# brayano/MultivarTV

Hardware: AMD Instinct MI355X
Metric: ADMM iters/sec on 512^3 fp64 mesh; achieved HBM GB/s vs peak at 1/2/4/8 GPUs (higher is better)
Workload: dtype f64; 1 GPU; 3D 512^3 fp64 mesh-TV ADMM, variant B (rcpp admm_update), lambda=1.0, fixed-iteration mode; theta_solver=spectral, nodes=134217728, edges=936381439, parallelism=single GPU

## Files before the change

### multivartv_amd/csrc/mvtv_admm3d.hip

```cpp
#include <algorithm>
#include <cstdlib>
#include <type_traits>

#include "mvtv_device.h"

namespace mvtv {

namespace e3d {
constexpr int TX = 64;
}

struct Edge3dArgs {
    Geom g;
    const double* theta;
    double* edges;
    const double* theta_old;
    double* g_alpha;
    double* g_u;
    const double* g_uprev;
    double* partials;
    double t_old, c_old, t_new;
    double t, c_prev;
    const AdmmCtl* ctl;
    int tiles_x, tiles_y, zchunk, nblocks;
// ... 316 lines not shown
    return pick(std::integral_constant<int, 256>{});
}

struct Fused3dArgs {
    Geom g;
    const double* theta;
    const double* z_old;
    double* z_new;
    const double* theta_old;
    double* g_alpha;
    double* g_u;
    const double* g_uprev;
    double* partials;
    double t_old, c_old, t_new, c_prev;
    const AdmmCtl* ctl;
    int tiles_x, tiles_y, zchunk, nblocks, zlo, zhi;
    int tpz;
    int xcd;
    int fold;
};

namespace f3a {
constexpr int IW = 65, IH = 15, TY = IH - 1, NT = 1024;
}

template <int NB, int ORD>
__host__ __device__ constexpr int f3a_nimg() {
    int n = 0;
    for (int k = 0; k < NB; ++k)
        if ((sprime_mask(block_code(k, 3, ORD), 3) & 3) != 0) ++n;
    return n;
}
template <int NB, int ORD>
__host__ __device__ constexpr int f3a_slot(int k) {
    int n = 0;
    for (int j = 0; j < k; ++j)
        if ((sprime_mask(block_code(j, 3, ORD), 3) & 3) != 0) ++n;
    return (sprime_mask(block_code(k, 3, ORD), 3) & 3) != 0 ? n : -1;
}

template <int ORD, int UM, bool DTH, int NB, bool TW>
__device__ __forceinline__ void admm3a_tile(const Fused3dArgs& a, double* __restrict__ szr, double (&red)[7], int X0,
                                            int Yh, int z0, int z1, double t_old, double c_old, double t_new,
                                            double c_prev, double rho_f) {
    constexpr int P = 3, NC = 8, IW = f3a::IW, IH = f3a::IH, NI = f3a_nimg<NB, ORD>();
    static_assert(!TW || twin_block(NB, P, ORD) >= 0, "twin blocks");
    const Geom& g = a.g;
    const int wv = int(threadIdx.x) >> 6, ln = int(threadIdx.x) & 63;
    const bool hcol = wv == IH;
    const int row = hcol ? ln : wv;
    const int col = hcol ? 0 : ln + 1;
    const int x = hcol ? X0 - 1 : X0 + ln, y = Yh + row;
    const int m0 = int(g.m[0]), m1 = int(g.m[1]), m2 = int(g.m[2]);
    const bool active = row < IH;
    const bool cell = active && x >= 0 && y >= 0 && x < m0 && y < m1;
    const bool inner = cell && !hcol && row > 0;
    const uint32_t pl = uint32_t(m0) * uint32_t(m1);
    const int xc = min(max(x, 0), m0 - 1), yc = min(max(y, 0), m1 - 1);
    const uint32_t xo[2] = {uint32_t(xc), uint32_t(min(xc + 1, m0 - 1))};
    const uint32_t yo[2] = {uint32_t(yc) * uint32_t(m0), uint32_t(min(yc + 1, m1 - 1)) * uint32_t(m0)};
    const uint32_t ixy = yo[0] + xo[0];
    const bool okx = x > 0, oky = y > 0;
    const bool hrow = row == 0;
    auto sidx = [&](int buf, int slot, int r, int c) { return ((buf * NI + slot) * IH + r) * IW + c; };

    auto load_theta = [&](double (&th)[4], int e) {
        const uint32_t zo = uint32_t(e) * pl;
#pragma unroll
        for (int q = 0; q < 4; ++q) th[q] = cell ? a.theta[zo + yo[q >> 1] + xo[q & 1]] : 0.0;
    };
    auto load_z = [&](double (&zo)[NB], int e) {
        const uint32_t i = uint32_t(e) * pl + ixy;
        static_for<0, NB>([&](auto kc) {
            constexpr int k = decltype(kc)::value;
            constexpr int S = sprime_mask(block_code(k, P, ORD), P);
            const bool need = cell && (!hrow || (S & 2)) && (!hcol || (S & 1));
            if constexpr (TW && twin_of(k, P, ORD) != k) zo[k] = 0.0;
            else zo[k] = need ? a.z_old[eix(g, k, i)] : 0.0;
        });
    };
    auto edge_cell = [&](int e, const double (&th0)[4], const double (&th1)[4], const double (&zo)[NB],
                         double (&zn)[NB], bool own) {
        const uint32_t i = uint32_t(e) * pl + ixy;
        double v[NC];
#pragma unroll
        for (int q = 0; q < 4; ++q) {
            v[q] = th0[q];
            v[q | 4] = th1[q];
        }
        if constexpr (DTH)
            if (own) red[3] = fmax(red[3], fabs(v[0] - a.theta_old[i]));
#pragma unroll
// ... 37 lines not shown
        constexpr int SI = S & 3;
        constexpr int sl = f3a_slot<NB, ORD>(k);
        qa = 0.0;
        qu = 0.0;
#pragma unroll
        for (int q = 0; q < 4; ++q) {
            if ((q & ~SI) != 0) continue;
            double v;
            if (q == 0) {
                v = own_z;
            } else {
                const bool ok = (!(q & 1) || okx) && (!(q & 2) || oky);
                if constexpr (sl >= 0) v = ok ? szr[sidx(buf, sl, row - ((q >> 1) & 1), col - (q & 1))] : 0.0;
                else v = 0.0;
            }
            const bool neg = __builtin_popcount(q) & 1;
            const double cl = clampd(v, t_new);
            const double al = v - cl;
            qa = neg ? qa - al : qa + al;
            qu = neg ? qu + cl : qu - cl;
        }
    };
    double qa_prev = 0.0, qu_prev = 0.0;
    double th0[4], th1[4], zo[NB], zn[NB];
    if (z0 > 0) {
        load_theta(th0, z0 - 1);
        load_theta(th1, z0);
        load_z(zo, z0 - 1);
        edge_cell(z0 - 1, th0, th1, zo, zn, false);
        to_image(1, zn);
        lds_barrier();
        if (inner) {
            static_for<0, NB>([&](auto kc) {
                constexpr int k = decltype(kc)::value;
                constexpr int S = sprime_mask(block_code(k, P, ORD), P);
                if constexpr ((S & 4) != 0 && !(TW && twin_of(k, P, ORD) != k)) {
                    constexpr double mk = TW ? double(twin_count(k, NB, P, ORD)) : 1.0;
                    double qa, qu;
                    plane_q(kc, 1, zn[k], qa, qu);
                    qa_prev = fma(mk * g.w[k], qa, qa_prev);
                    qu_prev = fma(mk * g.w[k], qu, qu_prev);
                }
            });
        }
        lds_barrier();
    }
    load_theta(th0, z0);
    load_theta(th1, min(z0 + 1, m2 - 1));
    load_z(zo, z0);
    double gp = inner ? __builtin_nontemporal_load(a.g_uprev + uint32_t(z0) * pl + ixy) : 0.0;
    for (int e = z0; e < z1; ++e) {
        const int buf = (e - z0) & 1;
        edge_cell(e, th0, th1, zo, zn, inner);
        to_image(buf, zn);
        double nth[4], nzo[NB], ngp = 0.0;
        if (e + 1 < z1) {
            load_theta(nth, min(e + 2, m2 - 1));
            load_z(nzo, e + 1);
            ngp = inner ? __builtin_nontemporal_load(a.g_uprev + uint32_t(e + 1) * pl + ixy) : 0.0;
        } else {
#pragma unroll
            for (int q = 0; q < 4; ++q) nth[q] = 0.0;
#pragma unroll
            for (int k = 0; k < NB; ++k) nzo[k] = 0.0;
        }
        lds_barrier();
        if (inner) {
            double ga = 0.0, gu = 0.0, na = 0.0, nu = 0.0;
            static_for<0, NB>([&](auto kc) {
                constexpr int k = decltype(kc)::value;
                constexpr int S = sprime_mask(block_code(k, P, ORD), P);
                if constexpr (!(TW && twin_of(k, P, ORD) != k)) {
                    constexpr double mk = TW ? double(twin_count(k, NB, P, ORD)) : 1.0;
                    const double wk = mk * g.w[k];
                    double qa, qu;
                    plane_q(kc, buf, zn[k], qa, qu);
                    ga = fma(wk, qa, ga);
                    gu = fma(wk, qu, gu);
                    if constexpr ((S & 4) != 0) {
                        na = fma(wk, qa, na);
                        nu = fma(wk, qu, nu);
                    }
                }
            });
            ga -= qa_prev;
            gu -= qu_prev;
            qa_prev = na;
            qu_prev = nu;
            const uint32_t i = uint32_t(e) * pl + ixy;
            __builtin_nontemporal_store(a.fold ? rho_f * (ga + gu) : ga, a.g_alpha + i);
            __builtin_nontemporal_store(gu, a.g_u + i);
            const double gpc = c_prev * gp;
            const double db = gu - gpc, da = ga + gpc;
            red[4] = fma(gu, gu, red[4]);
            red[5] = fma(db, db, red[5]);
            red[6] = fma(da, da, red[6]);
        }
#pragma unroll
        for (int q = 0; q < 4; ++q) {
            th0[q] = th1[q];
            th1[q] = nth[q];
        }
#pragma unroll
        for (int k = 0; k < NB; ++k) zo[k] = nzo[k];
        gp = ngp;
    }
}

template <int ORD, int UM, bool DTH, int NB, bool TW>
__global__ __launch_bounds__(f3a::NT) void k_admm3a(const Fused3dArgs a) {
    constexpr int NT = f3a::NT, NI = f3a_nimg<NB, ORD>();
    double t_old = a.t_old, c_old = a.c_old, t_new = a.t_new, c_prev = a.c_prev, rho_f = 0.0;
    if (a.ctl) {
        if (a.ctl->done) return;
        t_old = a.ctl->t_z;
        c_old = a.ctl->c_prev;
        t_new = a.ctl->t_next;
        c_prev = a.ctl->c_prev;
        rho_f = a.ctl->rho;
    }
    __shared__ double szr[2 * NI * f3a::IH * f3a::IW];
    double red[7] = {0.0, 0.0, 0.0, 0.0, 0.0, 0.0, 0.0};
    const int bid = a.xcd ? int((blockIdx.x & 7) * (gridDim.x >> 3) + (blockIdx.x >> 3)) : int(blockIdx.x);
    const bool valid = bid < a.nblocks;
    if (valid) {
        const int tz = bid / a.tpz, rem = bid - tz * a.tpz;
        const int z0 = a.zlo + tz * a.zchunk, z1 = min(a.zhi, z0 + a.zchunk);
        const int tyi = rem / a.tiles_x, txi = rem - tyi * a.tiles_x;
        admm3a_tile<ORD, UM, DTH, NB, TW>(a, szr, red, txi * 64, tyi * f3a::TY - 1, z0, z1, t_old, c_old, t_new,
                                          c_prev, rho_f);
    }
#pragma unroll
    for (int off = 32; off > 0; off >>= 1) {
#pragma unroll
        for (int k = 0; k < 7; ++k) {
            const double o = __shfl_down(red[k], off, 64);
            red[k] = k == 3 ? fmax(red[k], o) : red[k] + o;
        }
    }
    __shared__ double rs[NT / 64][7];
    const int w = threadIdx.x >> 6;
    __syncthreads();
    if ((threadIdx.x & 63) == 0)
        for (int k = 0; k < 7; ++k) rs[w][k] = valid ? red[k] : 0.0;
    __syncthreads();
    if (threadIdx.x < 7) {
        const int k = threadIdx.x;
        double acc = rs[0][k];
        for (int ww = 1; ww < NT / 64; ++ww) acc = k == 3 ? fmax(acc, rs[ww][k]) : acc + rs[ww][k];
        a.partials[blockIdx.x * 7 + k] = acc;
    }
}

// ... 48 lines not shown
    a.zchunk = (nzp + nz - 1) / nz;
    nz = (nzp + a.zchunk - 1) / a.zchunk;
    a.nblocks = tiles * nz;
    return a;
}
}

bool fused2d_ok(const Geom& g);
hipError_t launch_admm2d(const Geom& g, int order, int umode, hipStream_t s, const double* theta, const double* z_old,
                         double* z_new, double t_old, double c_old, double t_new, double c_prev,
                         const double* theta_old, double* g_alpha, double* g_u, const double* g_uprev,
                         double* partials, int* nparts, const AdmmCtl* ctl, bool fold);

bool fused3d_ok(const Geom& g) {
    if (g.p == 2) return fused2d_ok(g);
    if (g.p != 3 || probe_env("MVTV_F3D_OFF")) return false;
    const Fused3dArgs a = f3d_args(g);
    return ((a.nblocks + 7) / 8 * 8) * 7 <= kMaxCgBlocks * kMaxRed;
}

hipError_t launch_admm3d(const Geom& g, int order, int umode, hipStream_t s, const double* theta, const double* z_old,
                         double* z_new, double t_old, double c_old, double t_new, double c_prev,
                         const double* theta_old, double* g_alpha, double* g_u, const double* g_uprev,
                         double* partials, int* nparts, const AdmmCtl* ctl, bool fold, bool twin) {
    if (fold && ((g.p != 2 && g.p != 3) || !ctl)) return hipErrorInvalidValue;
    if (twin && (g.p != 3 || !twin_weights_equal(g, order)))
        return hipErrorInvalidValue;
    if (g.p == 2)
        return launch_admm2d(g, order, umode, s, theta, z_old, z_new, t_old, c_old, t_new, c_prev, theta_old, g_alpha,
                             g_u, g_uprev, partials, nparts, ctl, fold);
    Fused3dArgs a = f3d_args(g);
    a.theta = theta;
    a.z_old = z_old;
    a.z_new = z_new;
    a.theta_old = theta_old;
    a.g_alpha = g_alpha;
    a.g_u = g_u;
    a.g_uprev = g_uprev;
    a.partials = partials;
    a.t_old = t_old;
    a.c_old = c_old;
    a.t_new = t_new;
    a.c_prev = c_prev;
    a.ctl = ctl;
    a.fold = fold ? 1 : 0;
    const int grid = (a.nblocks + 7) / 8 * 8;
    *nparts = grid;
    const bool dth = theta_old != nullptr;
    auto go = [&](auto kern) {
        klaunch(kern, dim3(grid), dim3(f3a::NT), 0, s, a);
        return hipGetLastError();
    };
    auto pick = [&](auto ordc, auto nbc, auto twc) {
        constexpr int O = decltype(ordc)::value, NB = decltype(nbc)::value;
        constexpr bool T = decltype(twc)::value;
        if (umode == U_EXPLICIT)
            return dth ? go(k_admm3a<O, U_EXPLICIT, true, NB, T>) : go(k_admm3a<O, U_EXPLICIT, false, NB, T>);
        return dth ? go(k_admm3a<O, U_FROM_Z, true, NB, T>) : go(k_admm3a<O, U_FROM_Z, false, NB, T>);
    };
    using std::integral_constant;
    using T1 = integral_constant<bool, true>;
    using T0 = integral_constant<bool, false>;
    if (order == 0)
        return twin ? pick(integral_constant<int, 0>{}, integral_constant<int, 7>{}, T1{})
                    : pick(integral_constant<int, 0>{}, integral_constant<int, 7>{}, T0{});
    if (g.nb == 6)
        return twin ? pick(integral_constant<int, 1>{}, integral_constant<int, 6>{}, T1{})
                    : pick(integral_constant<int, 1>{}, integral_constant<int, 6>{}, T0{});
    return twin ? pick(integral_constant<int, 1>{}, integral_constant<int, 7>{}, T1{})
                : pick(integral_constant<int, 1>{}, integral_constant<int, 7>{}, T0{});
}

__global__ __launch_bounds__(256) void k_edges_copy_block(const Geom g, double* __restrict__ edges, int kdst, int ksrc,
                                                          uint32_t i0, uint32_t i1) {
    for (uint32_t i = i0 + blockIdx.x * 256u + threadIdx.x; i < i1; i += gridDim.x * 256u)
        edges[eix(g, kdst, i)] = edges[eix(g, ksrc, i)];
}

// ... 1163 lines not shown
```

### multivartv_amd/csrc/mvtv_capi.cpp

```cpp
#include <cxxabi.h>
#include <dlfcn.h>
#include <hip/hip_runtime.h>

#include <algorithm>
#include <chrono>
#include <cmath>
#include <cstdio>
#include <cstdlib>
#include <complex>
#include <cstdint>
#include <cstring>
#include <memory>
#include <string>
#include <vector>

#include "mvtv/mvtv.h"
#include "mvtv_internal.h"
#include "mvtv_problem.h"

using namespace mvtv;

namespace mvtv {
thread_local std::string g_last_error;
}
// ... 25 lines not shown
        if (c == '<') ++depth;
        else if (c == '>') --depth;
        else if (depth == 0 && c == ' ') start = i + 1;
        else if (depth == 0 && c == '(' && s.compare(i, 21, "(anonymous namespace)") == 0) i += 20;
        else if (depth == 0 && c == '(') { end = i; break; }
    }
    s = s.substr(start, end - start);
    for (const char* prefix : {"mvtv::", "__device_stub__"})
        if (s.compare(0, std::strlen(prefix), prefix) == 0) s.erase(0, std::strlen(prefix));
    return s;
}

bool twin_ready(const mvtv_problem* P) {
    if (P->slab || !P->twin_ok || probe_env("MVTV_TWIN_OFF")) return false;
    if (!((P->g.p == 3 && P->f3d) || (P->g.p == 4 && P->f4d))) return false;
    return twin_weights_equal(P->g, P->order);
}

double twin_edges(const mvtv_problem* P) {
    double t = 0.0;
    for (int k = 0; k < P->g.nb; ++k)
        if (twin_of(k, P->g.p, P->order) != k) t += double(P->blk_len[k]);
    return t;
}

mvtv_status pick_zpair(mvtv_problem* P, bool track_theta, bool twin) {
    P->zpicked = true;
    const char* env = std::getenv("MVTV_ZPICK");
    if ((env && std::atoi(env) == 0) || P->g.p != 3 || P->g.N < (size_t(1) << 24) || !P->edges2) return MVTV_OK;
    const size_t ne = size_t(P->g.nb) * P->g.N, bytes = ne * sizeof(double);
    size_t fr = 0, tot = 0;
    if (hipMemGetInfo(&fr, &tot) != hipSuccess || fr < 3 * bytes + (size_t(16) << 30)) {
        (void)hipGetLastError();
        return MVTV_OK;
    }
    constexpr int K = 4, R = 3;
    double* cand[K] = {P->edges2, nullptr, nullptr, nullptr};
    double* tmp[3] = {nullptr, nullptr, nullptr};
    hipEvent_t ev[2] = {nullptr, nullptr};
    bool ok = true;
    auto hip = [&](hipError_t e) {
        if (e != hipSuccess) ok = false;
        return ok;
    };
    for (int i = 1; i < K && ok; ++i) hip(hipMalloc(reinterpret_cast<void**>(&cand[i]), bytes));
    for (int i = 0; i < 3 && ok; ++i) hip(hipMalloc(reinterpret_cast<void**>(&tmp[i]), size_t(P->g.N) * sizeof(double)));
// ... 794 lines not shown
        P->wmean = acc / double(P->g.N);
        for (uint32_t i = 0; i < P->g.N; ++i) acc2 += (wdiag[i] - P->wmean) * (wdiag[i] - P->wmean);
        P->wstd = std::sqrt(acc2 / double(P->g.N));
        P->wsum_own = P->wsum2_own = 0.0;
        for (uint32_t i = P->g.ibeg; i < P->g.iend; ++i) {
            P->wsum_own += wdiag[i];
            P->wsum2_own += wdiag[i] * wdiag[i];
        }
    } else {
        P->wmode = W_IDENTITY;
        P->wmean = 1.0;
        P->wstd = 0.0;
        P->wsum_own = P->wsum2_own = double(P->g.iend - P->g.ibeg);
    }
    HIP_TRY(hipStreamSynchronize(P->stream));
    return MVTV_OK;
}

mvtv_status mvtv_state_set(mvtv_problem* P, const double* theta, const double* u, double rho) {
    if (!P || !theta) return fail(MVTV_BAD_ARG, "null problem/theta");
    DeviceGuard dg(P->device);
    HIP_TRY(hipMemcpyAsync(P->theta, theta, size_t(P->g.N) * sizeof(double), hipMemcpyHostToDevice, P->stream));
    P->twin_ok = true;
    if (u) {
        MVTV_TRY(import_edges(P, u, P->edges));
        P->u_default = false;
        uint64_t off[kMaxBlocks + 1] = {0};
        for (int k = 0; k < P->g.nb; ++k) off[k + 1] = off[k] + P->blk_len[k];
        for (int k = 0; k < P->g.nb && P->twin_ok; ++k) {
            const int c = twin_of(k, P->g.p, P->order);
            if (c != k)
                P->twin_ok = P->blk_len[k] == P->blk_len[c] &&
                             std::memcmp(u + off[k], u + off[c], size_t(P->blk_len[k]) * sizeof(double)) == 0;
        }
    } else {
        P->u_default = true;
    }
    HIP_TRY(hipStreamSynchronize(P->stream));
    P->edge_mode = U_EXPLICIT;
    P->t_z = 0.0;
    P->c_state = 1.0;
    P->rho = rho;
    P->have_state = true;
    return MVTV_OK;
}

mvtv_status mvtv_state_get(mvtv_problem* P, double* theta, double* u, double* rho) {
    if (!P) return fail(MVTV_BAD_ARG, "null problem");
    MVTV_TRY(ensure_state(P));
    DeviceGuard dg(P->device);
    if (theta) {
        HIP_TRY(hipMemcpyAsync(theta, P->theta, size_t(P->g.N) * sizeof(double), hipMemcpyDeviceToHost, P->stream));
        HIP_TRY(hipStreamSynchronize(P->stream));
    }
    if (u) {
        if (P->u_default) return fail(MVTV_BAD_ARG, "u is the variant default and has not been formed yet");
        MVTV_TRY(export_edges(P, P->edges, u, P->edge_mode, P->t_z, P->c_state));
    }
    if (rho) *rho = P->rho;
    return MVTV_OK;
}

mvtv_status mvtv_admm_run(mvtv_problem* P, const mvtv_admm_opts* opts_in, double lambda, mvtv_admm_stats* stats) {
    if (!P || !opts_in) return fail(MVTV_BAD_ARG, "null problem/opts");
    MVTV_TRY(ensure_state(P));
    if (!(lambda >= 0.0)) return fail(MVTV_BAD_ARG, "lambda must be >= 0");
    const auto t0 = std::chrono::steady_clock::now();
    DeviceGuard dg(P->device);
    const mvtv_admm_opts& o = *opts_in;
    const int variant = o.variant;
    if (variant < 0 || variant > 2) return fail(MVTV_BAD_ARG, "variant");
    const double tol = variant_tol(o);
    const int max_counter = variant_maxc(o);
    const double rtol = o.pcg_rtol > 0 ? o.pcg_rtol : 1e-10;
    const int pcg_maxit = o.pcg_max_iter > 0 ? o.pcg_max_iter : 20000;
    const Launch L = P->L();
    const double N = double(P->g.N), E = double(P->E);
    if (o.theta_solver < MVTV_SOLVER_AUTO || o.theta_solver > MVTV_SOLVER_PCG_SPECTRAL)
        return fail(MVTV_BAD_ARG, "theta_solver");
// ... 62 lines not shown
        HIP_TRY(hipMemcpyAsync(P->edges2, P->edges, size_t(P->g.nb) * P->g.N * sizeof(double),
                               hipMemcpyDeviceToDevice, P->stream));
        std::swap(P->edges, P->edges2);
    }
    if (fused && probe_env("MVTV_GFLIP")) {
        HIP_TRY(hipMemcpyAsync(P->gu, P->guprev, size_t(P->g.N) * sizeof(double), hipMemcpyDeviceToDevice,
                               P->stream));
        std::swap(P->gu, P->guprev);
    }
    const bool twin = (fused || fused4) && twin_ready(P);
    struct TwinGuard {
        mvtv_problem* P;
        bool armed;
        ~TwinGuard() {
            if (!armed) return;
            (void)fill_twins(P->g, P->order, P->stream, P->edges);
            if (P->edges2) (void)fill_twins(P->g, P->order, P->stream, P->edges2);
            if (P->edges3) (void)fill_twins(P->g, P->order, P->stream, P->edges3);
            (void)hipStreamSynchronize(P->stream);
            (void)hipGetLastError();
        }
    } twin_guard{P, twin};
    if (P->timing && (fused || fused4)) P->twin_timed = twin;
    if (fused && spectral && nbuf == 2 && !P->zpicked) MVTV_TRY(pick_zpair(P, track_theta, twin));
    double dtheta = 0.0;
    if (track_theta) {
        if (!P->thold) MVTV_TRY(alloc(&P->thold, P->g.N));
        HIP_TRY(launch_fill(P->stream, P->thold, o.ymean - (variant == MVTV_VARIANT_CPP ? 0.1 : 1.0), P->g.N));
        HIP_TRY(launch_maxabsdiff(P->g, L, P->theta, P->thold, P->partials));
        HIP_TRY(launch_finalize(P->stream, P->partials, L.grid, 1, 1, 0, P->red, P->st));
        HIP_TRY(hipMemcpyAsync(P->host_red, P->red, sizeof(double), hipMemcpyDeviceToHost, P->stream));
        MVTV_TRY(P->sync());
        dtheta = P->host_red[0];
    }

    const bool first_runs = o.fixed_iters > 0 ? o.fixed_iters > 0
                                              : (variant == MVTV_VARIANT_RCPP ? true
                                                                              : (dtheta > tol && !(variant == MVTV_VARIANT_PY &&
                                                                                                   max_counter <= 0)));
    if (spectral && first_runs && !std::getenv("MVTV_ADMM_SYNC")) {
        AdmmCtl& c = *P->host_ctl;
        std::memset(&c, 0, sizeof(c));
        c.variant = variant;
        c.fixed_iters = o.fixed_iters > 0 ? o.fixed_iters : 0;
        c.max_counter = max_counter;
        c.lambda = lambda;
// ... 12 lines not shown
        HIP_TRY(hipMemcpyAsync(P->ctl, &c, sizeof(AdmmCtl), hipMemcpyHostToDevice, P->stream));
        double* gbuf[2] = {P->guprev, P->gu};
        double* ebuf[3] = {P->edges, P->edges2, P->edges3};
        const uint32_t m0 = (!P->slab && march_ok(P->g)) ? P->g.m[2] : P->g.m[0];
        const bool fold_path = fused ? (P->g.p == 2 || P->g.p == 3)
                                     : (P->g.p == 4 && P->e3d && P->g4 != nullptr && gather4_ok(P->g));
        const uint64_t fold_stride = (!P->slab && march_ok(P->g)) ? uint64_t(P->g.m[0]) * P->g.m[1] : 1;
        const bool fold = fold_path && variant == MVTV_VARIANT_RCPP && m0 >= 8 && m0 <= 4096 &&
                          (m0 & (m0 - 1)) == 0 && (fold_stride & (fold_stride - 1)) == 0 &&
                          !probe_env("MVTV_FOLD_OFF") && !probe_env("MVTV_DCT_LDS") && !probe_env("MVTV_DCT_MID");
        auto enqueue = [&](int j) -> mvtv_status {
            double* gp = gbuf[j & 1];
            double* gn = gbuf[(j + 1) & 1];
            const int um = j == 0 ? mode : U_FROM_Z;
            if (track_theta)
                HIP_TRY(hipMemcpyAsync(P->thold, P->theta, size_t(P->g.N) * sizeof(double), hipMemcpyDeviceToDevice,
                                       P->stream));
            MVTV_TRY(spectral_solve(P, sigma, P->oty, P->ga, rho, gp, rho, P->theta, P->ctl, 1.0, nullptr,
                                    fold && j > 0));
            if (fused) {
                int hh = P->tstart(MVTV_K_ADMM_FUSED);
                int npf = 0;
                HIP_TRY(launch_admm3d(P->g, P->order, um, P->stream, P->theta, ebuf[j % nbuf], ebuf[(j + 1) % nbuf], 0.0, 1.0,
                                      0.0, 1.0, track_theta ? P->thold : nullptr, P->ga, gn, gp, P->partials, &npf,
                                      P->ctl, fold, twin));
                P->tstop(hh);
                hh = P->tstart(MVTV_K_REDUCE);
                HIP_TRY(launch_finalize(P->stream, P->partials, npf, ER_N + GR_N, -(1 << ER_DTH), 0, P->red, P->st, 0.0,
                                        0, P->ctl, P->ctl, P->red));
                P->tstop(hh);
                return MVTV_OK;
            }
            if (fused4) {
                int hh = P->tstart(MVTV_K_ADMM_FUSED4);
                int npe = 0;
                HIP_TRY(launch_admm4a(P->g, P->order, um, P->stream, P->theta, ebuf[j % nbuf], ebuf[(j + 1) % nbuf], 0.0,
                                      1.0, 0.0, track_theta ? P->thold : nullptr, P->g4, P->partials, &npe, P->ctl,
                                      twin));
                P->tstop(hh);
                hh = P->tstart(MVTV_K_REDUCE);
                HIP_TRY(launch_finalize(P->stream, P->partials, npe, ER_N, 1, 0, P->red, P->st, 0.0, 0, P->ctl));
                P->tstop(hh);
                hh = P->tstart(MVTV_K_GATHER4B);
                int npg = 0;
                HIP_TRY(launch_gather4b(P->g, U_FROM_Z, P->stream, P->ga, gn, gp, 1.0, P->partials, &npg, P->ctl, P->g4,
                                        fold));
                P->tstop(hh);
                hh = P->tstart(MVTV_K_REDUCE);
// ... 20 lines not shown
            if (P->e3d)
                HIP_TRY(launch_gather3d(P->g, P->order, U_FROM_Z, P->stream, P->edges, 0.0, P->ga, gn, gp, 1.0,
                                        P->partials, &npg, P->ctl, P->g4, fold));
            else
                HIP_TRY(launch_gather(P->g, P->order, U_FROM_Z, L, P->edges, 0.0, P->ga, gn, gp, 1.0, P->partials,
                                      P->ctl));
            P->tstop(hh);
            P->tstop_b(hb);
            hh = P->tstart(MVTV_K_REDUCE);
            HIP_TRY(launch_finalize(P->stream, P->partials, npg, GR_N, 0, 0, P->red + ER_N, P->st, 0.0, 0, P->ctl, P->ctl,
                                    P->red));
            P->tstop(hh);
            return MVTV_OK;
        };
        const int limit = o.fixed_iters > 0 ? o.fixed_iters
                                            : (variant == MVTV_VARIANT_PY ? max_counter : max_counter + 1);
        int target = o.fixed_iters > 0 ? o.fixed_iters : (P->admm_hint > 0 ? P->admm_hint : 16);
        hipGraphExec_t gexec = nullptr;
        if (!P->timing && nbuf == 2 && P->g.N < (uint32_t(1) << 24) && admm_graph_enabled()) {
            const std::vector<const void*> key = {P->theta, P->oty, P->ga, P->thold, gbuf[0], gbuf[1], ebuf[0], ebuf[1],
                                                  reinterpret_cast<const void*>(uintptr_t(fold)),
                                                  reinterpret_cast<const void*>(uintptr_t(track_theta)),
                                                  reinterpret_cast<const void*>(uintptr_t(fused)),
                                                  reinterpret_cast<const void*>(uintptr_t(twin))};
            auto it = std::find_if(P->graphs.begin(), P->graphs.end(), [&](const auto& lg) { return lg.key == key; });
            if (it == P->graphs.end()) {
                mvtv_problem::LoopGraph lg;
                lg.key = key;
                hipGraph_t gr = nullptr;
                if (hipStreamBeginCapture(P->stream, hipStreamCaptureModeThreadLocal) == hipSuccess) {
                    const bool ok = enqueue(1) == MVTV_OK && enqueue(2) == MVTV_OK;
                    const bool ended = hipStreamEndCapture(P->stream, &gr) == hipSuccess;
                    if (ok && ended && gr && hipGraphInstantiate(&lg.exec, gr, nullptr, nullptr, 0) != hipSuccess)
                        lg.exec = nullptr;
                    if (gr) (void)hipGraphDestroy(gr);
                }
                (void)hipGetLastError();
                if (P->graphs.size() >= 4) {
                    if (P->graphs.front().exec) (void)hipGraphExecDestroy(P->graphs.front().exec);
                    P->graphs.erase(P->graphs.begin());
                }
                P->graphs.push_back(lg);
                it = P->graphs.end() - 1;
            }
            gexec = it->exec;
        }
        const bool use_graph = gexec != nullptr;
// ... 9 lines not shown
                mark.push_back(P->pending.size());
                MVTV_TRY(enqueue(enq++));
            }
            HIP_TRY(hipMemcpyAsync(P->host_ctl, P->ctl, sizeof(AdmmCtl), hipMemcpyDeviceToHost, P->stream));
            HIP_TRY(hipStreamSynchronize(P->stream));
            if (c.done || enq >= limit) break;
            target = enq + std::max(4, enq / 4);
        }
        const int it_done = c.it;
        if (P->timing && it_done < int(mark.size()))
            for (size_t e = mark[size_t(it_done)]; e < P->pending.size(); ++e) P->pending[e].kid = -1;
        P->harvest();
        if (P->timing && fold) P->fold_fix += c.nfix;
        if (o.fixed_iters <= 0 && c.status == 0) P->admm_hint = it_done + 1;
        if (it_done & 1) std::swap(P->guprev, P->gu);
        if (fused && nbuf == 3) {
            P->edges = ebuf[it_done % 3];
            P->edges2 = ebuf[(it_done + 1) % 3];
            P->edges3 = ebuf[(it_done + 2) % 3];
        } else if (pingpong && (it_done & 1)) {
            std::swap(P->edges, P->edges2);
        }
        twin_guard.armed = false;
        if (twin) HIP_TRY(fill_twins(P->g, P->order, P->stream, P->edges));
        if (it_done > 0) P->edge_mode = U_FROM_Z;
        if (it_done > 0) P->t_z = c.t_z;
        P->c_state = c.c_prev;
        P->rho = c.rho;
        mvtv_admm_stats S{};
        S.iters = it_done;
        S.rho = c.rho;
        S.r_norm = c.r_norm;
        S.s_norm = c.s_norm;
        if (variant == MVTV_VARIANT_RCPP) {
            S.eps_pri = c.eps_pri;
            S.eps_dual = c.eps_dual;
        }
        S.dtheta_max = c.dtheta;
        S.theta_solver = MVTV_SOLVER_SPECTRAL;
        mvtv_status status = c.status ? MVTV_MAXITER : MVTV_OK;
        if (status == MVTV_MAXITER) {
            if (variant == MVTV_VARIANT_CPP) fail(status, "Failed to converge!");
            else if (variant == MVTV_VARIANT_RCPP && o.verbose) std::printf("ADMM reached max_counter at lambda = %g\n", lambda);
        }
        if (o.verbose) std::printf("Lambda= %g, Counter = %d\n", lambda, c.counter);
        S.status = status;
        S.seconds = std::chrono::duration<double>(std::chrono::steady_clock::now() - t0).count();
// ... 139 lines not shown
                    rho_next = 0.1 * rho;
                    c_next = 10.0;
                }
                rho_next = double(int(rho_next));
            }
        } else {
            dtheta = R[ER_DTH];
        }
        S.r_norm = r_norm;
        S.dtheta_max = dtheta;
        std::swap(gprev, gnew);
        c_prev = c_next;
        rho = rho_next;
        if (variant == MVTV_VARIANT_RCPP) sigma = rho;
        if (status == MVTV_MAXITER) break;
        if (variant == MVTV_VARIANT_RCPP && o.fixed_iters <= 0 && counter > max_counter) {
            if (o.verbose) std::printf("ADMM reached max_counter at lambda = %g\n", lambda);
            status = MVTV_MAXITER;
            break;
        }
    }
    P->harvest();
    twin_guard.armed = false;
    if (twin) {
        HIP_TRY(fill_twins(P->g, P->order, P->stream, P->edges));
        HIP_TRY(hipStreamSynchronize(P->stream));
    }
    if (o.verbose) std::printf("Lambda= %g, Counter = %d\n", lambda, counter);
    if (gprev != P->guprev) std::swap(P->guprev, P->gu);
    P->edge_mode = mode;
    P->t_z = t_z;
    P->c_state = c_prev;
    P->rho = rho;
    S.iters = it;
    S.theta_solver = spectral ? MVTV_SOLVER_SPECTRAL : (pcg_spec ? MVTV_SOLVER_PCG_SPECTRAL : MVTV_SOLVER_PCG);
    S.rho = rho;
    S.status = status;
    S.seconds = std::chrono::duration<double>(std::chrono::steady_clock::now() - t0).count();
    if (stats) *stats = S;
    return status;
}

mvtv_status mvtv_admm(mvtv_problem* P, const mvtv_admm_opts* opts, double lambda, double* theta_inout,
                      double* u_inout, double* rho_inout, mvtv_admm_stats* stats) {
    if (!P || !opts || !theta_inout) return fail(MVTV_BAD_ARG, "null problem/opts/theta");
    const double rho0 = rho_inout ? *rho_inout : lambda / 5.0;
    MVTV_TRY(mvtv_state_set(P, theta_inout, u_inout, rho0));
    mvtv_status s = mvtv_admm_run(P, opts, lambda, stats);
    if (s != MVTV_OK && s != MVTV_MAXITER) return s;
    mvtv_status g = mvtv_state_get(P, theta_inout, u_inout, rho_inout);
// ... 391 lines not shown
    }
    double b = 0.0;
    switch (kid) {
        case MVTV_K_EDGE_UPDATE: b = 8.0 * (N + 2.0 * E); break;
        case MVTV_K_GATHER:
            b = P->g4 ? 8.0 * (E + 4.0 * N) : 8.0 * (E + 3.0 * N);
            break;
        case MVTV_K_GATHER4B: b = 8.0 * 7.0 * N; break;
        case MVTV_K_PCG_INIT:
            b = 8.0 * (((P->g.p == 3 && P->fused3d) ? 5.0 : 6.0) + w) * N;
            break;
        case MVTV_K_PCG_APPLY: b = 8.0 * ((2.0 + w) * N); break;
        case MVTV_K_PCG_UPDATE: b = 8.0 * ((6.0 + w) * N); break;
        case MVTV_K_PCG_DIRECTION: b = 8.0 * ((3.0 + w) * N); break;
        case MVTV_K_PCG_FUSED:
            b = 8.0 * N * (4.0 + w + (P->launches[kid] > 0 ? 2.0 * double(P->pcg_xmoves) / double(P->launches[kid]) : 0.0));
            break;
        case MVTV_K_DCT_FIRST: b = 8.0 * 4.0 * N; break;
        case MVTV_K_DCT_FOLD:
            b = 8.0 * N * (3.0 + (P->launches[kid] > 0 ? double(P->fold_fix) / double(P->launches[kid]) : 0.0));
            break;
        case MVTV_K_DCT: b = 8.0 * 2.0 * N; break;
        case MVTV_K_ADMM_FUSED:
            b = 8.0 * (4.0 * N + 2.0 * (P->twin_timed ? E - twin_edges(P) * own : E));
            break;
        case MVTV_K_ADMM_FUSED4:
            b = 8.0 * (5.0 * N + 2.0 * (P->twin_timed ? E - twin_edges(P) * own : E));
            break;
        default: b = 0.0;
    }
    if (total_ms) *total_ms = P->ms[kid];
    if (launches) *launches = P->launches[kid];
    if (bytes) *bytes = b;
    return MVTV_OK;
}

const char* mvtv_kernel_name(int32_t kid) {
    static const char* names[MVTV_K_COUNT] = {"edge_update", "gather_Dt", "pcg_init", "pcg_apply_A",
                                               "pcg_update", "pcg_direction", "reduce", "other", "pcg_fused3d",
                                               "dct_first", "dct", "admm_fused", "gather4_b", "dct_first_fold",
                                               "admm_fused4"};
    return (kid >= 0 && kid < MVTV_K_COUNT) ? names[kid] : "?";
}

void mvtv_launch_log_enable(int32_t on) {
    static thread_local std::unique_ptr<LaunchRec[]> ring;
    LaunchLog& L = g_launch_log;
// ... 33 lines not shown
```

### multivartv_amd/csrc/mvtv_internal.h

```cpp
#pragma once
#include <stdint.h>

#include <hip/hip_ext.h>
#include <hip/hip_runtime.h>

#include <cstdlib>

namespace mvtv {

inline const char* probe_env(const char* name) {
#ifdef MVTV_PROBES
    return std::getenv(name);
#else
    (void)name;
    return nullptr;
#endif
}

inline bool probe_flag(const char* name) {
    const char* e = probe_env(name);
    return e && std::atoi(e) != 0;
}

struct FastDiv {
// ... 235 lines not shown
bool march_ok(const Geom& g);
hipError_t launch_march(const SpecPlan& sp, const Geom& g, hipStream_t s, bool bwd, double* x, double sigma, double w0,
                        const AdmmCtl* ctl = nullptr, const int32_t* skip = nullptr);
bool dct_pcg_fusable(const Geom& g, size_t partial_words);
bool dct_radix_plan(uint32_t m, int* rad, int* nrad);
hipError_t launch_dct_pass(const SpecPlan& sp, const Geom& g, hipStream_t s, int mode, int d, const double* in,
                           const double* ga, double ca, const double* gb, double cb, double* out, double sigma,
                           double w0, const AdmmCtl* ctl = nullptr, uint32_t q_off = 0, double inv_n = 0.0,
                           const int32_t* skip = nullptr, const PcgFuse* pf = nullptr, bool fold = false);
hipError_t launch_tri_slab(const SpecPlan& sp, const Geom& og, hipStream_t s, int phase, double* x, double* coef,
                           const double* lr, uint32_t chunk, int lo_ext, int hi_ext, double scale,
                           const AdmmCtl* ctl, double sigma = 1.0, double w0 = 1.0, const int32_t* skip = nullptr);
bool tri_slab_ok(uint32_t n);
int tri_slab_ncoef();
hipError_t launch_tri_iface(const SpecPlan& sp, const Geom& og, hipStream_t s, double* coef_in, double* lr_out,
                            uint32_t chunk, int G, int rank, uint32_t mg, const AdmmCtl* ctl, double sigma = 1.0,
                            double w0 = 1.0, const int32_t* skip = nullptr);
bool edge3d_ok(const Geom& g);
bool fused3d_ok(const Geom& g);
hipError_t launch_admm3d(const Geom& g, int order, int umode, hipStream_t s, const double* theta, const double* z_old,
                         double* z_new, double t_old, double c_old, double t_new, double c_prev,
                         const double* theta_old, double* g_alpha, double* g_u, const double* g_uprev,
                         double* partials, int* nparts, const AdmmCtl* ctl = nullptr, bool fold = false,
                         bool twin = false);
hipError_t launch_edges_copy_block(const Geom& g, hipStream_t s, double* edges, int kdst, int ksrc, uint32_t i0 = 0,
                                   uint32_t i1 = 0xffffffffu);
hipError_t fill_twins(const Geom& g, int order, hipStream_t s, double* edges, uint32_t i0 = 0, uint32_t i1 = 0xffffffffu);
hipError_t launch_edge3d(const Geom& g, int order, int umode, hipStream_t s, const double* theta, double* edges,
                         double t_old, double c_old, double t_new, const double* theta_old, double* partials,
                         int* nparts, const AdmmCtl* ctl = nullptr);
hipError_t launch_gather3d(const Geom& g, int order, int umode, hipStream_t s, const double* edges, double t,
                           double* g_alpha, double* g_u, const double* g_uprev, double c_prev, double* partials,
                           int* nparts, const AdmmCtl* ctl = nullptr, double* scratch4 = nullptr, bool fold = false);
bool gather4_ok(const Geom& g);
bool fused4_ok(const Geom& g);
hipError_t launch_admm4a(const Geom& g, int order, int umode, hipStream_t s, const double* theta, const double* z_old,
                         double* z_new, double t_old, double c_old, double t_new, const double* theta_old,
                         double* scratch4, double* partials, int* nparts, const AdmmCtl* ctl = nullptr, bool twin = false);
hipError_t launch_gather4b(const Geom& g, int umode, hipStream_t s, double* g_alpha, double* g_u, const double* g_uprev,
                           double c_prev, double* partials, int* nparts, const AdmmCtl* ctl, double* scratch4,
                           bool fold = false);
hipError_t launch_gather4a_ghost(const Geom& g, int order, hipStream_t s, const double* edges, double* scratch4,
                                 const AdmmCtl* ctl);
hipError_t launch_gather_index(hipStream_t s, const double* theta, const int64_t* idx, int64_t n, double* out);

hipError_t launch_nearest(hipStream_t s, int p, const uint32_t* m, const double* axes, const double* axes_host_span,
                          const double* data, int64_t n, uint32_t* key, int64_t* idx_out);
// ... 5 lines not shown
```

### multivartv_amd/csrc/mvtv_problem.h

```cpp
#pragma once
#include <hip/hip_runtime.h>

#include <algorithm>
#include <string>
#include <vector>

#include "mvtv/mvtv.h"
#include "mvtv_internal.h"

namespace mvtv {
extern thread_local std::string g_last_error;

inline mvtv_status fail(mvtv_status s, const std::string& msg) {
    g_last_error = msg;
    return s;
}
}

#define HIP_TRY(expr)                                                                                 \
    do {                                                                                              \
        hipError_t _e = (expr);                                                                       \
        if (_e != hipSuccess)                                                                         \
            return mvtv::fail(_e == hipErrorOutOfMemory ? MVTV_OUT_OF_MEMORY : MVTV_HIP_ERROR,        \
                              std::string(#expr) + ": " + hipGetErrorString(_e));                     \
// ... 65 lines not shown
    double wmean = 1.0;
    double wstd = 0.0;
    double wsum_own = 0.0, wsum2_own = 0.0;
    double* pcg_s = nullptr;
    double* pcg_t = nullptr;
    AdmmCtl* ctl = nullptr;
    AdmmCtl* host_ctl = nullptr;
    int admm_hint = 0;
    struct LoopGraph {
        std::vector<const void*> key;
        hipGraphExec_t exec = nullptr;
    };
    std::vector<LoopGraph> graphs;

    bool slab = false;
    int64_t m_global = 0, zb = 0, ze = 0;
    int g_lo = 0, g_hi = 0;
    double* slab_iface = nullptr;
    hipStream_t comm_stream = nullptr;

    bool have_state = false;
    bool u_default = true;
    bool twin_ok = true;
    bool twin_timed = false;
    int edge_mode = U_EXPLICIT;
    double t_z = 0.0, c_state = 1.0, rho = 0.0;

    bool timing = false;
    struct Pending {
        hipEvent_t a, b;
        int kid;
    };
    std::vector<Pending> pending;
    std::vector<hipEvent_t> ev_pool;
    double ms[MVTV_K_COUNT] = {0};
    int64_t launches[MVTV_K_COUNT] = {0};
    int64_t fold_fix = 0;
    int64_t pcg_xmoves = 0;

    Launch L() const { return Launch{stream, grid}; }

    hipEvent_t get_event() {
        if (!ev_pool.empty()) {
            hipEvent_t e = ev_pool.back();
            ev_pool.pop_back();
            return e;
        }
// ... 47 lines not shown
```

Before: 188.1 iters/s.

## Compute dual residual from theta stencil and defer twin edge filling

Adds an optional kernel variant that computes the dual residual by applying D^T D to theta through an LDS theta image, instead of reading the previous g_u array. This removes one full-mesh read from the fused ADMM kernel at the cost of extra LDS traffic and arithmetic. Separately, twin edge filling after an ADMM run becomes lazy and happens only when edges are exported or a non-twin path runs, which avoids a kernel and a stream sync per call. The stencil path is enabled only through an environment variable.

```diff
diff --git a/multivartv_amd/csrc/mvtv_admm3d.hip b/multivartv_amd/csrc/mvtv_admm3d.hip
--- a/multivartv_amd/csrc/mvtv_admm3d.hip
+++ b/multivartv_amd/csrc/mvtv_admm3d.hip
@@ -362,6 +362,7 @@
 
 namespace f3a {
 constexpr int IW = 65, IH = 15, TY = IH - 1, NT = 1024;
+constexpr int SW = IW + 1, SH = IH + 1;
 }
 
 template <int NB, int ORD>
@@ -379,12 +380,13 @@
     return (sprime_mask(block_code(k, 3, ORD), 3) & 3) != 0 ? n : -1;
 }
 
-template <int ORD, int UM, bool DTH, int NB, bool TW>
-__device__ __forceinline__ void admm3a_tile(const Fused3dArgs& a, double* __restrict__ szr, double (&red)[7], int X0,
-                                            int Yh, int z0, int z1, double t_old, double c_old, double t_new,
-                                            double c_prev, double rho_f) {
+template <int ORD, int UM, bool DTH, int NB, bool TW, bool SD>
+__device__ __forceinline__ void admm3a_tile(const Fused3dArgs& a, double* __restrict__ szr, double* __restrict__ sth,
+                                            double (&red)[7], int X0, int Yh, int z0, int z1, double t_old,
+                                            double c_old, double t_new, double c_prev, double rho_f) {
     constexpr int P = 3, NC = 8, IW = f3a::IW, IH = f3a::IH, NI = f3a_nimg<NB, ORD>();
     static_assert(!TW || twin_block(NB, P, ORD) >= 0, "twin blocks");
+    static_assert(!SD || !DTH, "the stencil dual is variant B's (no theta_old)");
     const Geom& g = a.g;
     const int wv = int(threadIdx.x) >> 6, ln = int(threadIdx.x) & 63;
     const bool hcol = wv == IH;
@@ -404,10 +406,33 @@
     const bool hrow = row == 0;
     auto sidx = [&](int buf, int slot, int r, int c) { return ((buf * NI + slot) * IH + r) * IW + c; };
 
+    const bool ldth = SD ? active : cell;
     auto load_theta = [&](double (&th)[4], int e) {
         const uint32_t zo = uint32_t(e) * pl;
 #pragma unroll
-        for (int q = 0; q < 4; ++q) th[q] = cell ? a.theta[zo + yo[q >> 1] + xo[q & 1]] : 0.0;
+        for (int q = 0; q < 4; ++q) th[q] = ldth ? a.theta[zo + yo[q >> 1] + xo[q & 1]] : 0.0;
+    };
+    auto tidx = [&](int buf, int r, int c) { return (buf * f3a::SH + r) * f3a::SW + c; };
+    auto theta_to_image = [&](int buf, const double (&th)[4]) {
+        if (!active) return;
+        sth[tidx(buf, row, col)] = th[0];
+        if (col == IW - 1) sth[tidx(buf, row, col + 1)] = th[1];
+        if (row == IH - 1) {
+            sth[tidx(buf, row + 1, col)] = th[2];
+            if (col == IW - 1) sth[tidx(buf, row + 1, col + 1)] = th[3];
+        }
+    };
+    auto dtd_plane = [&](int buf, const double (&th)[4], double& q, double& ip) {
+        const double tw = sth[tidx(buf, row, col - 1)], ts = sth[tidx(buf, row - 1, col)];
+        const double tsw = sth[tidx(buf, row - 1, col - 1)], tse = sth[tidx(buf, row - 1, col + 1)];
+        const double tnw = sth[tidx(buf, row + 1, col - 1)];
+        const double l1c = 2.0 * th[0] - ts - th[2];
+        const double l1w = 2.0 * tw - tsw - tnw;
+        const double l1e = 2.0 * th[1] - tse - th[3];
+        const double a0 = 2.0 * th[0] - tw - th[1];
+        const double a01 = 2.0 * l1c - l1w - l1e;
+        q = fma(g.cS[7], a01, fma(g.cS[6], l1c, fma(g.cS[5], a0, g.cS[4] * th[0])));
+        ip = fma(g.cS[3], a01, fma(g.cS[2], l1c, g.cS[1] * a0));
     };
     auto load_z = [&](double (&zo)[NB], int e) {
         const uint32_t i = uint32_t(e) * pl + ixy;
@@ -491,6 +516,7 @@
         }
     };
     double qa_prev = 0.0, qu_prev = 0.0;
+    double q_lo = 0.0, q_c = 0.0, ip_c = 0.0;
     double th0[4], th1[4], zo[NB], zn[NB];
     if (z0 > 0) {
         load_theta(th0, z0 - 1);
@@ -498,7 +524,18 @@
         load_z(zo, z0 - 1);
         edge_cell(z0 - 1, th0, th1, zo, zn, false);
         to_image(1, zn);
+        if constexpr (SD) {
+            theta_to_image(0, th0);
+            theta_to_image(1, th1);
+        }
         lds_barrier();
+        if constexpr (SD) {
+            if (inner) {
+                double ip_lo;
+                dtd_plane(0, th0, q_lo, ip_lo);
+                dtd_plane(1, th1, q_c, ip_c);
+            }
+        }
         if (inner) {
             static_for<0, NB>([&](auto kc) {
                 constexpr int k = decltype(kc)::value;
@@ -517,16 +554,25 @@
     load_theta(th0, z0);
     load_theta(th1, min(z0 + 1, m2 - 1));
     load_z(zo, z0);
-    double gp = inner ? __builtin_nontemporal_load(a.g_uprev + uint32_t(z0) * pl + ixy) : 0.0;
+    if constexpr (SD) {
+        if (z0 == 0) {
+            theta_to_image(1, th0);
+            lds_barrier();
+            if (inner) dtd_plane(1, th0, q_c, ip_c);
+        }
+    }
+    double gp = 0.0;
+    if constexpr (!SD) gp = inner ? __builtin_nontemporal_load(a.g_uprev + uint32_t(z0) * pl + ixy) : 0.0;
     for (int e = z0; e < z1; ++e) {
         const int buf = (e - z0) & 1;
         edge_cell(e, th0, th1, zo, zn, inner);
         to_image(buf, zn);
+        if constexpr (SD) theta_to_image(buf, th1);
         double nth[4], nzo[NB], ngp = 0.0;
         if (e + 1 < z1) {
             load_theta(nth, min(e + 2, m2 - 1));
             load_z(nzo, e + 1);
-            ngp = inner ? __builtin_nontemporal_load(a.g_uprev + uint32_t(e + 1) * pl + ixy) : 0.0;
+            if constexpr (!SD) ngp = inner ? __builtin_nontemporal_load(a.g_uprev + uint32_t(e + 1) * pl + ixy) : 0.0;
         } else {
 #pragma unroll
             for (int q = 0; q < 4; ++q) nth[q] = 0.0;
@@ -559,11 +605,24 @@
             const uint32_t i = uint32_t(e) * pl + ixy;
             __builtin_nontemporal_store(a.fold ? rho_f * (ga + gu) : ga, a.g_alpha + i);
             __builtin_nontemporal_store(gu, a.g_u + i);
-            const double gpc = c_prev * gp;
-            const double db = gu - gpc, da = ga + gpc;
             red[4] = fma(gu, gu, red[4]);
-            red[5] = fma(db, db, red[5]);
-            red[6] = fma(da, da, red[6]);
+            if constexpr (SD) {
+                double q_hi, ip_hi;
+                dtd_plane(buf, th1, q_hi, ip_hi);
+                double dd = ip_c;
+                if (e > 0) dd += q_c - q_lo;
+                if (e < m2 - 1) dd += q_c - q_hi;
+                const double db = ga - dd;
+                red[5] = fma(db, db, red[5]);
+                q_lo = q_c;
+                q_c = q_hi;
+                ip_c = ip_hi;
+            } else {
+                const double gpc = c_prev * gp;
+                const double db = gu - gpc, da = ga + gpc;
+                red[5] = fma(db, db, red[5]);
+                red[6] = fma(da, da, red[6]);
+            }
         }
 #pragma unroll
         for (int q = 0; q < 4; ++q) {
@@ -576,7 +635,7 @@
     }
 }
 
-template <int ORD, int UM, bool DTH, int NB, bool TW>
+template <int ORD, int UM, bool DTH, int NB, bool TW, bool SD = false>
 __global__ __launch_bounds__(f3a::NT) void k_admm3a(const Fused3dArgs a) {
     constexpr int NT = f3a::NT, NI = f3a_nimg<NB, ORD>();
     double t_old = a.t_old, c_old = a.c_old, t_new = a.t_new, c_prev = a.c_prev, rho_f = 0.0;
@@ -589,6 +648,11 @@
         rho_f = a.ctl->rho;
     }
     __shared__ double szr[2 * NI * f3a::IH * f3a::IW];
+    double* sth = nullptr;
+    if constexpr (SD) {
+        __shared__ double sth_img[2 * f3a::SH * f3a::SW];
+        sth = sth_img;
+    }
     double red[7] = {0.0, 0.0, 0.0, 0.0, 0.0, 0.0, 0.0};
     const int bid = a.xcd ? int((blockIdx.x & 7) * (gridDim.x >> 3) + (blockIdx.x >> 3)) : int(blockIdx.x);
     const bool valid = bid < a.nblocks;
@@ -596,8 +660,8 @@
         const int tz = bid / a.tpz, rem = bid - tz * a.tpz;
         const int z0 = a.zlo + tz * a.zchunk, z1 = min(a.zhi, z0 + a.zchunk);
         const int tyi = rem / a.tiles_x, txi = rem - tyi * a.tiles_x;
-        admm3a_tile<ORD, UM, DTH, NB, TW>(a, szr, red, txi * 64, tyi * f3a::TY - 1, z0, z1, t_old, c_old, t_new,
-                                          c_prev, rho_f);
+        admm3a_tile<ORD, UM, DTH, NB, TW, SD>(a, szr, sth, red, txi * 64, tyi * f3a::TY - 1, z0, z1, t_old, c_old,
+                                              t_new, c_prev, rho_f);
     }
 #pragma unroll
     for (int off = 32; off > 0; off >>= 1) {
@@ -692,8 +756,9 @@
 hipError_t launch_admm3d(const Geom& g, int order, int umode, hipStream_t s, const double* theta, const double* z_old,
                          double* z_new, double t_old, double c_old, double t_new, double c_prev,
                          const double* theta_old, double* g_alpha, double* g_u, const double* g_uprev,
-                         double* partials, int* nparts, const AdmmCtl* ctl, bool fold, bool twin) {
+                         double* partials, int* nparts, const AdmmCtl* ctl, bool fold, bool twin, bool sdual) {
     if (fold && ((g.p != 2 && g.p != 3) || !ctl)) return hipErrorInvalidValue;
+    if (sdual && (g.p != 3 || !ctl || theta_old || g.ibeg != 0 || g.iend != g.N)) return hipErrorInvalidValue;
     if (twin && (g.p != 3 || !twin_weights_equal(g, order)))
         return hipErrorInvalidValue;
     if (g.p == 2)
@@ -724,6 +789,9 @@
     auto pick = [&](auto ordc, auto nbc, auto twc) {
         constexpr int O = decltype(ordc)::value, NB = decltype(nbc)::value;
         constexpr bool T = decltype(twc)::value;
+        if (sdual)
+            return umode == U_EXPLICIT ? go(k_admm3a<O, U_EXPLICIT, false, NB, T, true>)
+                                       : go(k_admm3a<O, U_FROM_Z, false, NB, T, true>);
         if (umode == U_EXPLICIT)
             return dth ? go(k_admm3a<O, U_EXPLICIT, true, NB, T>) : go(k_admm3a<O, U_EXPLICIT, false, NB, T>);
         return dth ? go(k_admm3a<O, U_FROM_Z, true, NB, T>) : go(k_admm3a<O, U_FROM_Z, false, NB, T>);
diff --git a/multivartv_amd/csrc/mvtv_capi.cpp b/multivartv_amd/csrc/mvtv_capi.cpp
--- a/multivartv_amd/csrc/mvtv_capi.cpp
+++ b/multivartv_amd/csrc/mvtv_capi.cpp
@@ -71,6 +71,19 @@
     for (int k = 0; k < P->g.nb; ++k)
         if (twin_of(k, P->g.p, P->order) != k) t += double(P->blk_len[k]);
     return t;
+}
+
+bool dual_stencil_wanted() {
+    const char* env = std::getenv("MVTV_DUAL_STENCIL");
+    return env && std::atoi(env) != 0;
+}
+
+mvtv_status settle_twins(mvtv_problem* P) {
+    if (!P->twin_stale) return MVTV_OK;
+    HIP_TRY(fill_twins(P->g, P->order, P->stream, P->edges));
+    HIP_TRY(hipStreamSynchronize(P->stream));
+    P->twin_stale = false;
+    return MVTV_OK;
 }
 
 mvtv_status pick_zpair(mvtv_problem* P, bool track_theta, bool twin) {
@@ -911,6 +924,7 @@
     DeviceGuard dg(P->device);
     HIP_TRY(hipMemcpyAsync(P->theta, theta, size_t(P->g.N) * sizeof(double), hipMemcpyHostToDevice, P->stream));
     P->twin_ok = true;
+    P->twin_stale = false;
     if (u) {
         MVTV_TRY(import_edges(P, u, P->edges));
         P->u_default = false;
@@ -944,6 +958,7 @@
     }
     if (u) {
         if (P->u_default) return fail(MVTV_BAD_ARG, "u is the variant default and has not been formed yet");
+        MVTV_TRY(settle_twins(P));
         MVTV_TRY(export_edges(P, P->edges, u, P->edge_mode, P->t_z, P->c_state));
     }
     if (rho) *rho = P->rho;
@@ -1052,6 +1067,10 @@
         }
     } twin_guard{P, twin};
     if (P->timing && (fused || fused4)) P->twin_timed = twin;
+    const bool sdual = fused && P->g.p == 3 && !P->slab && variant == MVTV_VARIANT_RCPP && spectral &&
+                       !std::getenv("MVTV_ADMM_SYNC") && dual_stencil_wanted();
+    if (P->timing && fused) P->sdual_timed = sdual;
+    if (!twin) MVTV_TRY(settle_twins(P));
     if (fused && spectral && nbuf == 2 && !P->zpicked) MVTV_TRY(pick_zpair(P, track_theta, twin));
     double dtheta = 0.0;
     if (track_theta) {
@@ -1110,8 +1129,8 @@
                 int hh = P->tstart(MVTV_K_ADMM_FUSED);
                 int npf = 0;
                 HIP_TRY(launch_admm3d(P->g, P->order, um, P->stream, P->theta, ebuf[j % nbuf], ebuf[(j + 1) % nbuf], 0.0, 1.0,
-                                      0.0, 1.0, track_theta ? P->thold : nullptr, P->ga, gn, gp, P->partials, &npf,
-                                      P->ctl, fold, twin));
+                                      0.0, 1.0, track_theta ? P->thold : nullptr, P->ga, gn, sdual ? nullptr : gp,
+                                      P->partials, &npf, P->ctl, fold, twin, sdual));
                 P->tstop(hh);
                 hh = P->tstart(MVTV_K_REDUCE);
                 HIP_TRY(launch_finalize(P->stream, P->partials, npf, ER_N + GR_N, -(1 << ER_DTH), 0, P->red, P->st, 0.0,
@@ -1178,7 +1197,8 @@
                                                   reinterpret_cast<const void*>(uintptr_t(fold)),
                                                   reinterpret_cast<const void*>(uintptr_t(track_theta)),
                                                   reinterpret_cast<const void*>(uintptr_t(fused)),
-                                                  reinterpret_cast<const void*>(uintptr_t(twin))};
+                                                  reinterpret_cast<const void*>(uintptr_t(twin)),
+                                                  reinterpret_cast<const void*>(uintptr_t(sdual))};
             auto it = std::find_if(P->graphs.begin(), P->graphs.end(), [&](const auto& lg) { return lg.key == key; });
             if (it == P->graphs.end()) {
                 mvtv_problem::LoopGraph lg;
@@ -1234,7 +1254,7 @@
             std::swap(P->edges, P->edges2);
         }
         twin_guard.armed = false;
-        if (twin) HIP_TRY(fill_twins(P->g, P->order, P->stream, P->edges));
+        if (twin && it_done > 0) P->twin_stale = true;
         if (it_done > 0) P->edge_mode = U_FROM_Z;
         if (it_done > 0) P->t_z = c.t_z;
         P->c_state = c.c_prev;
@@ -1420,10 +1440,7 @@
     }
     P->harvest();
     twin_guard.armed = false;
-    if (twin) {
-        HIP_TRY(fill_twins(P->g, P->order, P->stream, P->edges));
-        HIP_TRY(hipStreamSynchronize(P->stream));
-    }
+    if (twin && it > 0) P->twin_stale = true;
     if (o.verbose) std::printf("Lambda= %g, Counter = %d\n", lambda, counter);
     if (gprev != P->guprev) std::swap(P->guprev, P->gu);
     P->edge_mode = mode;
@@ -1861,7 +1878,7 @@
             break;
         case MVTV_K_DCT: b = 8.0 * 2.0 * N; break;
         case MVTV_K_ADMM_FUSED:
-            b = 8.0 * (4.0 * N + 2.0 * (P->twin_timed ? E - twin_edges(P) * own : E));
+            b = 8.0 * ((P->sdual_timed ? 3.0 : 4.0) * N + 2.0 * (P->twin_timed ? E - twin_edges(P) * own : E));
             break;
         case MVTV_K_ADMM_FUSED4:
             b = 8.0 * (5.0 * N + 2.0 * (P->twin_timed ? E - twin_edges(P) * own : E));
diff --git a/multivartv_amd/csrc/mvtv_internal.h b/multivartv_amd/csrc/mvtv_internal.h
--- a/multivartv_amd/csrc/mvtv_internal.h
+++ b/multivartv_amd/csrc/mvtv_internal.h
@@ -281,7 +281,7 @@
                          double* z_new, double t_old, double c_old, double t_new, double c_prev,
                          const double* theta_old, double* g_alpha, double* g_u, const double* g_uprev,
                          double* partials, int* nparts, const AdmmCtl* ctl = nullptr, bool fold = false,
-                         bool twin = false);
+                         bool twin = false, bool sdual = false);
 hipError_t launch_edges_copy_block(const Geom& g, hipStream_t s, double* edges, int kdst, int ksrc, uint32_t i0 = 0,
                                    uint32_t i1 = 0xffffffffu);
 hipError_t fill_twins(const Geom& g, int order, hipStream_t s, double* edges, uint32_t i0 = 0, uint32_t i1 = 0xffffffffu);
diff --git a/multivartv_amd/csrc/mvtv_problem.h b/multivartv_amd/csrc/mvtv_problem.h
--- a/multivartv_amd/csrc/mvtv_problem.h
+++ b/multivartv_amd/csrc/mvtv_problem.h
@@ -111,7 +111,9 @@
     bool have_state = false;
     bool u_default = true;
     bool twin_ok = true;
+    bool twin_stale = false;
     bool twin_timed = false;
+    bool sdual_timed = false;
     int edge_mode = U_EXPLICIT;
     double t_z = 0.0, c_state = 1.0, rho = 0.0;
 
```

Measured after the change: 188.5 iters/s (median of 5 runs). About the same (+0.2%).
